# kowaalczyk/reformer-tts

Measured on AMD Instinct MI355X. Metric: mel-frames/sec training step, LJSpeech-shape batch, higher is better.
Workload: dtype bf16; 1 GPU; config/baseline.yml full Reformer-TTS training step (enc 3 / dec 3 layers, d=512, LSH 8 rounds, buckets 64/128), per-GPU batch 12, text 200->256, mel 1024x80; global_batch=12, parallelism=dp1, reversible_recompute=full

## Files before the change

### include/rtts.h

```cpp
#ifndef RTTS_H
#define RTTS_H

#include <stdint.h>

#ifdef __cplusplus
extern "C" {
#endif

#define RTTS_VERSION 1

int rtts_version(void);
const char* rtts_last_error(void);

int rtts_lsh_hash_sort(const void* qk, int64_t ld_qk, const float* rotations, int rot_rows,
                       int B, int H, int T, int dh, int n_hashes, int bucket_size,
                       int32_t* buckets, int32_t* st, int32_t* undo, void* stream);
int rtts_lsh_hash_sort_launches(int T);

int rtts_lsh_hash_sort_hf(const void* qk, int64_t ld_qk, const float* rotations, const uint8_t* mask,
                          int B, int H, int T, int dh, int n_hashes, int chunk, int n_buckets,
                          int32_t* buckets, int32_t* st, int32_t* undo, void* stream);

int rtts_lsh_attn_fwd(const void* qk, const void* v, int64_t ld, const int32_t* st, const uint8_t* mask,
                      int B, int H, int T, int dh, int n_hashes, int bucket_size, int causal,
// ... 109 lines not shown
int rtts_bn_act_bwd_sums(const float* y, const void* dz, int dz_halo, const float* mean, const float* rstd, const float* gamma,
                         const float* beta, int act, float drop_p, uint32_t seed, const uint32_t* seed_dev, int B, int L, int halo, int C,
                         float* sums, float* dgamma, float* dbeta, float* partial_ws, void* stream);
int rtts_bn_act_bwd_apply(const float* y, const void* dz, int dz_halo, const float* mean, const float* rstd, const float* gamma,
                          const float* beta, int act, float drop_p, uint32_t seed, const uint32_t* seed_dev, int B, int L, int halo, int C,
                          const float* sums, int64_t count, void* dy, int dy_lead, int64_t dy_rows, void* stream);
int rtts_tts_loss(const float* raw, const float* post, int64_t ld_mel, const float* tgt, const float* mask, const float* stop,
                  int64_t ld_stop, const float* tstop, int rows, int NM, int kind, float pos_weight, float w_raw, float w_post,
                  float w_stop, float* d_raw, float* d_post, int64_t ld_grad, float* d_stop, float* losses, float* partial_ws,
                  int padded_len, int valid_len, const float* res, int64_t ld_res, int halo, int dpost_lead, int64_t dpost_rows,
                  int64_t tgt_batch_stride, const int32_t* valid_len_dev, int64_t mask_batch_stride, int64_t tstop_batch_stride,
                  void* stream);
int rtts_heads_grad(const float* d_raw, const float* d_post, int dpost_lead, const float* dx0, int64_t ld_dx0, const float* d_stop,
                    int B, int L, int halo, int n_mels, int width, float* dheads, const float* scale_dev, void* stream);

#define RTTS_SEGMENTS_MAX 12
enum { RTTS_SEG_COPY_F32 = 0, RTTS_SEG_COPY_BF16 = 1, RTTS_SEG_ADD_F32 = 2, RTTS_SEG_CAST_F32_BF16 = 3 };
typedef struct {
    void* dst;
    const void* src;
    int64_t count;
    int32_t kind, reserved;
} rtts_segment;
int rtts_segments(const rtts_segment* jobs, int n, void* stream);

int rtts_pe_add(const void* y, const float* table, const float* alpha, float drop_p, uint32_t seed, const uint32_t* seed_dev,
                int T, int64_t M, int d, float* out, void* stream);
int rtts_pe_dalpha(const float* dy, const float* table, float drop_p, uint32_t seed, const uint32_t* seed_dev, int T, int64_t M,
                   int d, float* dalpha, float* partial_ws, void* stream);
int rtts_relu_drop(void* h, float drop_p, uint32_t seed, const uint32_t* seed_dev, int64_t n, void* stream);

int rtts_batch_masks(const int64_t* phonemes, int64_t ph_stride, int B, int Lp, int Lp_pad, const float* loss_mask, int64_t lm_bstride,
                     int64_t lm_rstride, int Lm, int Lm_pad, int n_mels, int64_t* pad_phonemes, uint8_t* phoneme_mask,
                     uint8_t* phoneme_pad_mask, uint8_t* frame_mask, void* stream);

int rtts_embedding_fwd(const int64_t* ids, const float* E, int rows, int C, int n_embeddings, float drop_p, uint32_t seed,
                       const uint32_t* seed_dev, float* out, void* stream);
int rtts_embedding_bwd(const int64_t* ids, const float* dx, int rows, int C, int n_embeddings, int padding_idx, float* dE,
                       float drop_p, uint32_t seed, const uint32_t* seed_dev, void* stream);
int rtts_embedding_bwd_strided(const int64_t* ids, const float* dx, int64_t batch_stride, int64_t row_stride, int L, int rows, int C,
                               int n_embeddings, int padding_idx, float* dE, float drop_p, uint32_t seed, const uint32_t* seed_dev, void* stream);

int rtts_gemm_tn(const void* a, int64_t lda, const void* b, int64_t ldb, int M, int N, int K, float* c, int64_t ldc,
                 int accumulate, float* slab_ws, int64_t slab_ws_floats, void* stream);

#define RTTS_GEMM_TN_MAX_GROUP 16
typedef struct {
    const void* a; int64_t lda;
    const void* b; int64_t ldb;
    float* c;      int64_t ldc;
    int32_t M, N, K, accumulate;
} rtts_gemm_tn_problem;
int rtts_gemm_tn_grouped(const rtts_gemm_tn_problem* problems, int n, float* slab_ws, int64_t slab_ws_floats, void* stream);

int rtts_gemm_nt(const void* a, int64_t lda, const void* w, int64_t ldw, int w_is_kn, int M, int N, int K, void* c,
                 int64_t ldc, const float* bias, int epilogue, const void* gate, int64_t ldg, float* colsum_partial,
                 void* stream);
int rtts_gemm_nt_partial_rows(int M, int N);
typedef struct {
    const void* a; int64_t lda;
    const void* w; int64_t ldw;
    void* c; int64_t ldc;
    const float* bias;
    const void* aux; int64_t ld_aux;
    float* aux_out;
    int32_t M, N, K, epilogue;
    int32_t T, H, accumulate, reserved;
} rtts_gemm_nt_problem;
#define RTTS_GEMM_NT_MAX_GROUP 4
int rtts_gemm_nt_grouped(const rtts_gemm_nt_problem* problems, int n, int w_is_kn, void* stream);
int rtts_debug_set_gemm_mode(int mode);
int64_t rtts_gemm_nt_gate_words(int M, int N);
int rtts_gemm_nt_gated(const void* a, int64_t lda, const void* w, int64_t ldw, int w_is_kn, int M, int N, int K, void* c,
                       int64_t ldc, const float* bias, int epilogue, uint64_t* gate_words, float* colsum_partial, void* stream);

int rtts_peak_copy(const void* src, void* dst, int64_t bytes, void* stream);
int rtts_comm_probe(const void* src, void* dst, int64_t bytes, int workgroups, int sleep, void* stream);
int rtts_debug_stamp(void* buf, int slot, void* stream);
int rtts_peak_mfma(float* sink, int workgroups, int iters, void* stream);

int rtts_sw_depthwise_k3(const float* x, const float* w, const float* bias, int B, int L, int C, void* y,
                         const float* edge_lo, const float* edge_hi, void* stream);
int rtts_sw_gate(const void* pw, const void* cond, int64_t ld_cond, int cond_offset, int upsample, int B, int L, int Lm, int C,
                 void* acts, void* stream);
int rtts_sw_coupling_inv(float* audio, int64_t ld_audio, const float* wn_out, int64_t rows, int half, void* stream);
int rtts_sw_depthwise_k3_seg(const float* x, const float* w, const float* bias, const int32_t* moff, int nseg, int upsample,
                             int64_t rows, int C, void* y, const float* edge_lo, const float* edge_hi, void* stream);
int rtts_sw_pack_mel(const float* mel, int64_t stride_b, int64_t stride_c, int64_t stride_t, int L, int n_mel, const int32_t* moff,
                     int nseg, int64_t rows, float* dst, int64_t ld_dst, void* stream);
int rtts_sw_coupling_inv1x1(const float* audio, int64_t ld_audio, const float* wn_out, int64_t ld_wn, const float* winv, int n,
                            int64_t rows, float* out, int64_t ld_out, void* stream);
int rtts_sw_coupling_fwd1x1(const float* x, int64_t ld_x, const float* wn_out, int64_t ld_wn, const float* w, int n_in, int n_early,
                            int64_t rows, float* out, int64_t ld_out, float* z, int64_t ld_z, int z_col, float* ls_row, void* stream);
int rtts_sw_nll_reduce(const float* z, int64_t ld_z, int C, const float* ls_row, const int32_t* moff, int nseg, int upsample, int64_t L,
                       int64_t rows, double* out, void* stream);
int rtts_sw_pack_audio(const float* src, int64_t n_src, const int64_t* start, const int32_t* moff, int nseg, int upsample, int C,
                       int64_t rows, float* dst, void* stream);
int rtts_sw_gate_bwd(const void* pw, const void* cond, int64_t ld_cond, int cond_offset, int upsample, int B, int L, int Lm, int C,
                     const void* dacts, void* dpw, void* dcond, int64_t ld_dcond, void* stream);
int rtts_sw_dwbn_bwd_partial_floats(int64_t rows, int C);
int rtts_sw_dwbn_bwd_sums(const float* h, const void* dy, const float* mean, const float* rstd, const float* gamma, const float* beta,
                          const float* w, int B, int L, int C, float* sums, float* partial_ws, void* stream);
int rtts_sw_dwbn_bwd_apply(const float* h, const void* dy, const float* mean, const float* rstd, const float* gamma, const float* beta,
                           const float* w, const float* sums, int B, int L, int C, float* dh, void* stream);
int rtts_sw_boundary_bwd_blocks(int64_t rows);
int rtts_sw_boundary_bwd(const float* x, int64_t ld_x, const float* wn_out, int64_t ld_wn, const float* w, int n_in, int n_early,
// ... 63 lines not shown
```

### reformer-tts_amd/_lib.py

```python
from __future__ import annotations

import ctypes as C
import os

_HERE = os.path.dirname(os.path.abspath(__file__))
LIB_PATH = os.environ.get("RTTS_LIB") or os.path.join(_HERE, "lib", "librtts_hip.so")

_i64, _i32, _vp, _f32, _u32 = C.c_int64, C.c_int, C.c_void_p, C.c_float, C.c_uint32

class GemmTnProblem(C.Structure):
    _fields_ = [("a", _vp), ("lda", _i64), ("b", _vp), ("ldb", _i64), ("c", _vp), ("ldc", _i64),
                ("M", C.c_int32), ("N", C.c_int32), ("K", C.c_int32), ("accumulate", C.c_int32)]


GEMM_TN_MAX_GROUP = 16


class GemmNtProblem(C.Structure):
    _fields_ = [("a", _vp), ("lda", _i64), ("w", _vp), ("ldw", _i64), ("c", _vp), ("ldc", _i64), ("bias", _vp), ("aux", _vp),
                ("ld_aux", _i64), ("aux_out", _vp), ("M", C.c_int32), ("N", C.c_int32), ("K", C.c_int32), ("epilogue", C.c_int32),
                ("T", C.c_int32), ("H", C.c_int32), ("accumulate", C.c_int32), ("reserved", C.c_int32)]


GEMM_NT_MAX_GROUP = 4


class ColsumJob(C.Structure):
    _fields_ = [("partial", _vp), ("out", _vp), ("nrows", C.c_int32), ("n", C.c_int32), ("ld", C.c_int32), ("reserved", C.c_int32)]


COLSUM_MAX_GROUP = 48


class Segment(C.Structure):
    _fields_ = [("dst", _vp), ("src", _vp), ("count", C.c_int64), ("kind", C.c_int32), ("reserved", C.c_int32)]


SEGMENTS_MAX = 12
SEG_COPY_F32, SEG_COPY_BF16, SEG_ADD_F32, SEG_CAST_F32_BF16 = 0, 1, 2, 3


class ConvPermJob(C.Structure):
    _fields_ = [("w", _vp), ("wp", _vp), ("Co", C.c_int32), ("Ci", C.c_int32), ("CP", C.c_int32), ("reserved", C.c_int32)]


CONV_PERM_MAX_GROUP = 8
SW_FACTOR_MAX_COUNT, SW_FACTOR_MAX_N = 16, 128

SIGNATURES = {
    "rtts_lsh_hash_sort": [_vp, _i64, _vp, _i32, _i32, _i32, _i32, _i32, _i32, _i32, _vp, _vp, _vp, _vp],
    "rtts_lsh_attn_fwd": [_vp, _vp, _i64, _vp, _vp, _i32, _i32, _i32, _i32, _i32, _i32, _i32, _vp, _vp, _f32, _u32, _vp, _vp],
    "rtts_lsh_hash_sort_launches": [_i32],
    "rtts_lsh_hash_sort_hf": [_vp, _i64, _vp, _vp, _i32, _i32, _i32, _i32, _i32, _i32, _i32, _vp, _vp, _vp, _vp],
    "rtts_lsh_attn_fwd_run_length": [_i32, _i32, _i32, _i32, _i32],
    "rtts_lsh_combine_fwd": [_vp, _vp, _i32, _i32, _i32, _i32, _i32, _vp, _i64, _vp, _vp],
    "rtts_lsh_bwd_delta": [_vp, _i64, _vp, _i64, _i32, _i32, _i32, _i32, _vp, _vp],
    "rtts_lsh_attn_bwd": [_vp, _vp, _i64, _vp, _vp, _vp, _i64, _vp, _vp, _i32, _i32, _i32, _i32, _i32, _i32, _i32, _vp, _vp, _vp, _f32, _u32, _vp,
                          _vp],
    "rtts_lsh_bwd_qk_slots": [],
    "rtts_lsh_attn_bwd_run_length": [_i32, _i32, _i32, _i32, _i32],
    "rtts_debug_set_walk": [_i32, _i32],
    "rtts_lsh_bwd_reduce": [_vp, _vp, _i32, _i32, _i32, _i32, _i32, _vp, _vp, _i64, _vp, _vp],
    "rtts_grad_clip_scale": [_vp, _i64, _f32, _f32, _vp, _vp, _vp],
    "rtts_ln_fwd": [_vp, _vp, _vp, _vp, _vp, _vp, _i32, _i32, _vp],
    "rtts_ln_bwd": [_vp, _vp, _vp, _vp, _vp, _vp, _vp, _vp, _vp, _i32, _i32, _vp, _vp, _f32, _u32, _vp, _vp],
    "rtts_ln_bwd_to": [_vp, _vp, _vp, _vp, _vp, _vp, _vp, _vp, _vp, _vp, _i32, _i32, _vp, _vp, _f32, _u32, _vp, _vp],
    "rtts_ln_bwd_join": [_vp, _vp, _vp, _vp, _vp, _vp, _vp, _vp, _vp, _vp, _vp, _i32, _i32, _vp, _vp, _f32, _u32, _vp, _vp],
    "rtts_cast_colsum": [_vp, _vp, _vp, _vp, _i32, _i32, _f32, _u32, _vp, _vp, _vp],
    "rtts_colsum_bf16": [_vp, _vp, _i64, _vp, _vp, _i32, _i32, _i32, _f32, _vp, _vp],
    "rtts_sum_streams": [_vp, _vp, _i64, _vp, _vp, _vp],
    "rtts_residual_epilogue": [_vp, _vp, _vp, _f32, _vp, _i64, _i32, _f32, _u32, _vp, _vp],
    "rtts_colsum_partial_rows": [_i32],
    "rtts_colsum_final_grouped": [C.POINTER(ColsumJob), _i32, _vp],
    "rtts_residual_ln": [_vp, _vp, _vp, _f32, _vp, _vp, _vp, _vp, _vp, _i32, _i32, _f32, _u32, _vp, _vp, _vp],
    "rtts_bias_act": [_vp, _vp, _i64, _i32, _i32, _vp],
    "rtts_cast_f32_bf16": [_vp, _vp, _i64, _vp],
    "rtts_xattn_fwd": [_vp, _i64, _vp, _i64, _vp, _i32, _i32, _i32, _i32, _i32, _vp, _i64, _vp, _f32, _u32, _vp, _vp],
    "rtts_xattn_bwd": [_vp, _i64, _vp, _i64, _vp, _vp, _i64, _vp, _vp, _i32, _i32, _i32, _i32, _i32, _vp, _i64, _vp, _f32, _u32, _vp, _vp, _vp],
    "rtts_xattn_key_chunks": [_i32],
    "rtts_xattn_bwd_key_chunks": [_i32, _i32],
    "rtts_xattn_probs_mean": [_vp, _i64, _vp, _i64, _vp, _vp, _i32, _i32, _i32, _i32, _i32, _vp, _i64, _vp],
    "rtts_sum_slabs": [_vp, _i32, _i64, _vp, _vp],
    "rtts_full_attn_max_t": [_i32],
    "rtts_full_attn_fwd": [_vp, _vp, _i64, _vp, _i32, _i32, _i32, _i32, _i32, _vp, _i64, _vp, _f32, _u32, _vp, _vp],
    "rtts_full_attn_bwd_workspace": [_i32, _i32, _i32, _i32],
    "rtts_full_attn_bwd": [_vp, _vp, _i64, _vp, _vp, _i64, _vp, _vp, _i32, _i32, _i32, _i32, _i32, _vp, _vp, _i64, _vp, _f32, _u32, _vp,
                           _vp],
    "rtts_conv1d_k5": [_vp, _i64, _vp, _i64, _i32, _i32, _i32, _i32, _vp, _i64, _vp, _i32, _vp],
    "rtts_to_halo": [_vp, _i64, _i64, _i32, _i32, _i32, _i32, _i32, _i32, _vp, _i32, _i64, _vp],
    "rtts_heads_grad": [_vp, _vp, _i32, _vp, _i64, _vp, _i32, _i32, _i32, _i32, _i32, _vp, _vp, _vp],
    "rtts_segments": [C.POINTER(Segment), _i32, _vp],
    "rtts_conv_w_perm": [_vp, _i32, _i32, _i32, _vp, _vp],
    "rtts_conv_dw_unperm": [_vp, _i32, _i32, _i32, _vp, _vp],
    "rtts_conv_w_perm_grouped": [C.POINTER(ConvPermJob), _i32, _vp],
    "rtts_conv_dw_unperm_grouped": [C.POINTER(ConvPermJob), _i32, _vp],
    "rtts_conv1d_k5_moments": [_vp, _i64, _vp, _i64, _i32, _i32, _i32, _vp, _i64, _i32, _i32, _i32, _vp, _vp],
    "rtts_bn_stats_from_partials": [_vp, _i32, _i32, _i32, _i32, _vp, _vp, _vp, _vp, _vp, _vp, _vp],
    "rtts_bn_stats": [_vp, _i32, _i32, _i32, _i32, _vp, _vp, _vp, _vp, _vp, _vp, _vp, _vp],
    "rtts_bn_act_fwd": [_vp, _vp, _vp, _vp, _vp, _i32, _f32, _u32, _vp, _i32, _i32, _i32, _i32, _vp, _i32, _i32, _i64, _vp],
    "rtts_bn_act_bwd": [_vp, _vp, _i32, _vp, _vp, _vp, _vp, _i32, _f32, _u32, _vp, _i32, _i32, _i32, _i32, _vp, _i32, _i64, _vp, _vp, _vp, _vp],
    "rtts_bn_moments": [_vp, _i32, _i32, _i32, _i32, _vp, _vp, _vp],
    "rtts_bn_from_moments": [_vp, _i64, _i32, _vp, _vp, _vp, _vp, _vp, _vp, _vp],
    "rtts_bn_act_bwd_sums": [_vp, _vp, _i32, _vp, _vp, _vp, _vp, _i32, _f32, _u32, _vp, _i32, _i32, _i32, _i32, _vp, _vp, _vp, _vp, _vp],
    "rtts_bn_act_bwd_apply": [_vp, _vp, _i32, _vp, _vp, _vp, _vp, _i32, _f32, _u32, _vp, _i32, _i32, _i32, _i32, _vp, _i64, _vp, _i32, _i64, _vp],
    "rtts_tts_loss": [_vp, _vp, _i64, _vp, _vp, _vp, _i64, _vp, _i32, _i32, _i32, _f32, _f32, _f32, _f32, _vp, _vp, _i64, _vp, _vp, _vp, _i32, _i32,
                      _vp, _i64, _i32, _i32, _i64, _i64, _vp, _i64, _i64, _vp],
    "rtts_pe_add": [_vp, _vp, _vp, _f32, _u32, _vp, _i32, _i64, _i32, _vp, _vp],
    "rtts_debug_stamp": [_vp, _i32, _vp],
    "rtts_batch_masks": [_vp, _i64, _i32, _i32, _i32, _vp, _i64, _i64, _i32, _i32, _i32, _vp, _vp, _vp, _vp, _vp],
    "rtts_pe_dalpha": [_vp, _vp, _f32, _u32, _vp, _i32, _i64, _i32, _vp, _vp, _vp],
    "rtts_relu_drop": [_vp, _f32, _u32, _vp, _i64, _vp],
    "rtts_embedding_bwd": [_vp, _vp, _i32, _i32, _i32, _i32, _vp, _f32, _u32, _vp, _vp],
    "rtts_embedding_bwd_strided": [_vp, _vp, _i64, _i64, _i32, _i32, _i32, _i32, _i32, _vp, _f32, _u32, _vp, _vp],
    "rtts_embedding_fwd": [_vp, _vp, _i32, _i32, _i32, _f32, _u32, _vp, _vp, _vp],
    "rtts_gemm_tn": [_vp, _i64, _vp, _i64, _i32, _i32, _i32, _vp, _i64, _i32, _vp, _i64, _vp],
    "rtts_gemm_tn_grouped": [C.POINTER(GemmTnProblem), _i32, _vp, _i64, _vp],
    "rtts_gemm_nt": [_vp, _i64, _vp, _i64, _i32, _i32, _i32, _i32, _vp, _i64, _vp, _i32, _vp, _i64, _vp, _vp],
    "rtts_gemm_nt_partial_rows": [_i32, _i32],
    "rtts_gemm_nt_grouped": [C.POINTER(GemmNtProblem), _i32, _i32, _vp],
    "rtts_debug_set_gemm_mode": [_i32],
    "rtts_gemm_nt_gate_words": [_i32, _i32],
    "rtts_gemm_nt_gated": [_vp, _i64, _vp, _i64, _i32, _i32, _i32, _i32, _vp, _i64, _vp, _i32, _vp, _vp, _vp],
    "rtts_peak_copy": [_vp, _vp, _i64, _vp],
    "rtts_comm_probe": [_vp, _vp, _i64, _i32, _i32, _vp],
    "rtts_peak_mfma": [_vp, _i32, _i32, _vp],
    "rtts_sw_depthwise_k3": [_vp, _vp, _vp, _i32, _i32, _i32, _vp, _vp, _vp, _vp],
    "rtts_sw_gate": [_vp, _vp, _i64, _i32, _i32, _i32, _i32, _i32, _i32, _vp, _vp],
    "rtts_sw_coupling_inv": [_vp, _i64, _vp, _i64, _i32, _vp],
    "rtts_sw_depthwise_k3_seg": [_vp, _vp, _vp, _vp, _i32, _i32, _i64, _i32, _vp, _vp, _vp, _vp],
    "rtts_sw_pack_mel": [_vp, _i64, _i64, _i64, _i32, _i32, _vp, _i32, _i64, _vp, _i64, _vp],
    "rtts_sw_coupling_inv1x1": [_vp, _i64, _vp, _i64, _vp, _i32, _i64, _vp, _i64, _vp],
    "rtts_sw_coupling_fwd1x1": [_vp, _i64, _vp, _i64, _vp, _i32, _i32, _i64, _vp, _i64, _vp, _i64, _i32, _vp, _vp],
    "rtts_sw_nll_reduce": [_vp, _i64, _i32, _vp, _vp, _i32, _i32, _i64, _i64, _vp, _vp],
    "rtts_sw_pack_audio": [_vp, _i64, _vp, _vp, _i32, _i32, _i32, _i64, _vp, _vp],
    "rtts_sw_gate_bwd": [_vp, _vp, _i64, _i32, _i32, _i32, _i32, _i32, _i32, _vp, _vp, _vp, _i64, _vp],
    "rtts_sw_dwbn_bwd_partial_floats": [_i64, _i32],
    "rtts_sw_dwbn_bwd_sums": [_vp, _vp, _vp, _vp, _vp, _vp, _vp, _i32, _i32, _i32, _vp, _vp, _vp],
    "rtts_sw_dwbn_bwd_apply": [_vp, _vp, _vp, _vp, _vp, _vp, _vp, _vp, _i32, _i32, _i32, _vp, _vp],
    "rtts_sw_boundary_bwd_blocks": [_i64],
    "rtts_sw_boundary_bwd": [_vp, _i64, _vp, _i64, _vp, _i32, _i32, _i64, _vp, _i64, _vp, _i64, _i32, _f32, _f32, _vp, _i64, _vp, _i64, _vp, _vp,
                             _vp],
    "rtts_sw_inv1x1_factor": [C.POINTER(_vp), C.POINTER(_i32), _i32, C.POINTER(_vp), _vp, _vp],
    "rtts_sw_draw_segments": [_vp, _i32, _i64, _vp, _vp, _i64, _vp, _i32, _vp, _i32, _vp, _u32, _vp, _i32, _i32, _i32, _i32, _i32, _vp, _vp, _i64,
                              _vp, _vp],
    "rtts_tts_collate": [_vp, _i64, _vp, _vp, _i64, _vp, _i32, _vp, _i32, _i32, _i32, _vp, _i32, _vp, _i32, _i32, _vp, _i32, _vp, _i32, _vp, _i32,
                         _vp, _f32, _u32, _vp],
    "rtts_infer_metrics_tiles": [_i32],
    "rtts_infer_metrics": [_vp, _i64, _i64, _i64, _i32, _vp, _vp, _i64, _i64, _i64, _vp, _i32, _vp, _vp, _vp, _i32, _i32, _i32, _i32, _vp, _vp, _vp,
                           _vp, _vp],
    "rtts_dtw_max_frames": [],
    "rtts_dtw_workspace_bytes": [_i32, _i32, _i32, _i32],
    "rtts_dtw_align": [_vp, _i64, _i64, _i64, _i32, _vp, _vp, _i64, _i64, _i64, _vp, _i32, _vp, _vp, _vp, _i32, _i32, _i32, _vp, _i32, _vp, _i64,
                       _i32, _vp, _vp, _vp, _vp],
    "rtts_adamw_step": [_vp, _vp, _vp, _vp, _vp, _i64, _vp, _vp, _f32, _f32, _f32, _f32, _vp, _vp],
    "rtts_mel_frames": [_i64, _i32],
    "rtts_mel_spectrogram": [_vp, C.POINTER(_i64), C.POINTER(_i64), _vp, _vp, _i32, _vp, _vp, _i32, _i32, _i32, _i32, _f32, _vp, _i64, _vp],
    "rtts_resample_len": [_i64, _i32, _i32],
    "rtts_resample": [_vp, _i32, _i32, C.POINTER(_i64), C.POINTER(_i64), _vp, _vp, _i32, _vp, _vp, _i32, _i32, _i32, _vp, _vp],
    "rtts_denoise": [_vp, C.POINTER(_i64), _vp, _i32, _vp, _vp, _vp, _f32, _i32, _i32, _vp, _vp],
    "rtts_gl_magnitudes": [_vp, _i64, _i64, _i64, _vp, C.POINTER(_i64), _vp, _i32, _vp, _i32, _i32, _i32, _vp, _i64, _vp],
    "rtts_gl_init": [_vp, _i64, C.POINTER(_i64), _vp, C.POINTER(_i64), _vp, _i32, _vp, _vp, _i32, _u32, _i32, _i32, _vp, _vp],
    "rtts_gl_step": [_vp, _vp, _f32, _vp, _i64, C.POINTER(_i64), _vp, C.POINTER(_i64), _vp, _i32, _vp, _vp, _i32, _i32, _vp, _vp],
}

_lib = None


class RttsError(RuntimeError):
    pass
# ... 82 lines not shown
```

### reformer-tts_amd/edges.py

```python
from __future__ import annotations

import threading
from typing import List

import torch

from . import _lib
from . import engine as _engine
from .engine import WEIGHT_EPOCH, _WS, _bf16, _grad, bf16_twin, cast_colsum, gemm, wgrad

from ._seeds import _seed_counter, seed_base


def _s() -> int:
    return torch.cuda.current_stream().cuda_stream


def _ws(device, c: int) -> torch.Tensor:
    key = ("edge", device, c, torch.cuda.current_stream(device).cuda_stream)
    if key not in _WS._cache:
        _WS._cache[key] = torch.empty((2 * 256 + 2) * c, dtype=torch.float32, device=device)
    return _WS._cache[key]


def _pad128(c: int) -> int:
    return -(-c // 128) * 128


class Halo:
    H, LEAD, TILE = 2, 8, 256

    def __init__(self, b: int, l: int):
        self.b, self.l = b, l
        self.p = l + 2 * self.H
        self.rows = b * self.p
        self.mp = -(-self.rows // self.TILE) * self.TILE
        self.alloc = self.mp + 2 * self.LEAD

    def new(self, c: int, device, dtype=torch.bfloat16) -> torch.Tensor:
        return torch.empty(self.alloc, c, dtype=dtype, device=device)

    def body(self, buf: torch.Tensor, shift: int = 0) -> torch.Tensor:
        return buf[self.LEAD + shift:self.LEAD + shift + self.mp]

    def valid(self, body: torch.Tensor) -> torch.Tensor:
        return body[:self.rows].view(self.b, self.p, -1)[:, self.H:self.H + self.l]


import os as _os
CONVS_PER_WGRAD_LAUNCH = int(_os.environ.get("RTTS_CONVS_PER_WGRAD", "4"))


def flush_conv_wgrad(queue=None) -> None:
    queue = _engine._queue() if queue is None else queue
    q = queue.conv_gemms
    wide = [p for p in q if p[0][7] % 256 == 0 and p[0][8] % 256 == 0]
    rest = [p for p in q if not (p[0][7] % 256 == 0 and p[0][8] % 256 == 0)]
    del q[:]
    for part in (wide, rest):
        while part:
            chunk = part[:_lib.GEMM_TN_MAX_GROUP]
            del part[:len(chunk)]
            arr = (_lib.GemmTnProblem * len(chunk))()
            for dst, (fields, _keep) in zip(arr, chunk):
                dst.a, dst.lda, dst.b, dst.ldb, dst.c, dst.ldc, dst.M, dst.N, dst.K, dst.accumulate = fields
            ws = _engine._slab_ws(chunk[0][1][0].device, queue.stream)
            _lib.call("rtts_gemm_tn_grouped", arr, len(chunk), ws.data_ptr(), ws.numel(), queue.stream)


def flush_conv_dw(queue=None) -> None:
    queue = _engine._queue() if queue is None else queue
    flush_conv_wgrad(queue)
    pending = list(queue.conv_items)
    del queue.conv_items[:]
    for chunk in _engine.launch_groups(pending, _lib.CONV_PERM_MAX_GROUP,
                                       lambda a, b: _engine.spans_overlap(a[4].data_ptr(), 20 * a[1] * a[2], b[4].data_ptr(), 20 * b[1] * b[2])):
        jobs = (_lib.ConvPermJob * len(chunk))()
        for j, (dwp, co, ci, cp, gw) in zip(jobs, chunk):
            j.w, j.wp, j.Co, j.Ci, j.CP = dwp.data_ptr(), gw.data_ptr(), co, ci, cp
        _lib.call("rtts_conv_dw_unperm_grouped", jobs, len(chunk), queue.stream)


class ConvK5:

    instances = None

    def __init__(self, conv: torch.nn.Conv1d):
        self.conv = conv
        self.co, self.ci = conv.out_channels, conv.in_channels
        self.cp = _pad128(self.ci)
        self.cop = _pad128(self.co)
        self._wp = None
        self._wp_version = None
        if ConvK5.instances is None:
            import weakref
            ConvK5.instances = weakref.WeakSet()
        ConvK5.instances.add(self)

    def _version(self):
        w = self.conv.weight
        return (w._version, WEIGHT_EPOCH[0], w.data_ptr())

    @staticmethod
    def refresh_all(device) -> None:
        stale = [c for c in (ConvK5.instances or ()) if c.conv.weight.device == device and c._wp_version != c._version()]
        for i in range(0, len(stale), _lib.CONV_PERM_MAX_GROUP):
            chunk = stale[i:i + _lib.CONV_PERM_MAX_GROUP]
            jobs = (_lib.ConvPermJob * len(chunk))()
            for j, c in zip(jobs, chunk):
                if c._wp is None or c._wp.device != device:
                    c._wp = torch.zeros(c.cop, 5 * c.cp, dtype=torch.bfloat16, device=device)
                j.w, j.wp, j.Co, j.Ci, j.CP = c.conv.weight.data_ptr(), c._wp.data_ptr(), c.co, c.ci, c.cp
            _lib.call("rtts_conv_w_perm_grouped", jobs, len(chunk), _s())
            for c in chunk:
                c._wp_version = c._version()

    def weight_perm(self) -> torch.Tensor:
        w = self.conv.weight
        ver = (w._version, WEIGHT_EPOCH[0], w.data_ptr())
        if self._wp is None or self._wp_version != ver or self._wp.device != w.device:
            if self._wp is None or self._wp.device != w.device:
                self._wp = torch.zeros(self.cop, 5 * self.cp, dtype=torch.bfloat16, device=w.device)
            _lib.call("rtts_conv_w_perm", w.data_ptr(), self.co, self.ci, self.cp, self._wp.data_ptr(), _s())
            self._wp_version = ver
        return self._wp

    def forward(self, xh: torch.Tensor, g: Halo, bias=None) -> torch.Tensor:
        y = torch.empty(g.mp, self.cop, dtype=torch.float32, device=xh.device)
        wp = self.weight_perm()
        _lib.call("rtts_conv1d_k5", g.body(xh).data_ptr(), self.cp, wp.data_ptr(), 5 * self.cp, 0, g.mp, self.cop, self.cp, y.data_ptr(),
                  self.cop, None if bias is None else bias.data_ptr(), 1, _s())
        return y

    def forward_moments(self, xh: torch.Tensor, g: Halo):
        y = torch.empty(g.mp, self.cop, dtype=torch.float32, device=xh.device)
        nrows = _lib.load().rtts_gemm_nt_partial_rows(g.mp, self.cop)
        if nrows <= 0:
            raise _lib.RttsError(f"rtts_conv1d_k5_moments: no tile shape for {g.mp} x {self.cop}")
        partial = torch.empty(nrows, 2 * self.cop, dtype=torch.float32, device=xh.device)
        _lib.call("rtts_conv1d_k5_moments", g.body(xh).data_ptr(), self.cp, self.weight_perm().data_ptr(), 5 * self.cp, g.mp, self.cop, self.cp,
                  y.data_ptr(), self.cop, g.b, g.l, g.H, partial.data_ptr(), _s())
        return y, partial, nrows

    def backward(self, dyh: torch.Tensor, xh: torch.Tensor, g: Halo, need_dx: bool = True, dx_f32: bool = False):
        dev = dyh.device
        dwp = torch.empty(self.cop, 5 * self.cp, dtype=torch.float32, device=dev)
        dyb = g.body(dyh)
        dwq = _engine._queue()
        for k in range(5):
            xs, ck = g.body(xh, k - 2), dwp[:, k * self.cp:(k + 1) * self.cp]
            dwq.conv_gemms.append(((dyb.data_ptr(), self.cop, xs.data_ptr(), self.cp, ck.data_ptr(), 5 * self.cp, g.mp, self.cop, self.cp, 0),
                              (dyh, xh, dwp)))
        if len(dwq.conv_gemms) >= 5 * CONVS_PER_WGRAD_LAUNCH:
            flush_conv_wgrad(dwq)
        dwq.conv_items.append((dwp, self.co, self.ci, self.cp, _grad(self.conv.weight)))
        if len(dwq.conv_items) >= _lib.CONV_PERM_MAX_GROUP:
            flush_conv_dw(dwq)
        else:
            from .engine import _queue_final_flush
            _queue_final_flush()
        if not need_dx:
            return None
        dx = torch.empty(g.mp, self.cp, dtype=torch.float32 if dx_f32 else torch.bfloat16, device=dev)
        _lib.call("rtts_conv1d_k5", dyb.data_ptr(), self.cop, self.weight_perm().data_ptr(), 5 * self.cp, 1, g.mp, self.cp, self.cop,
                  dx.data_ptr(), self.cp, None, int(dx_f32), _s())
        return dx


SYNC_BN = None
CONV_MOMENTS = _os.environ.get("RTTS_CONV_MOMENTS", "1") != "0"


class ConvBNAct:

    def __init__(self, conv, bn, act: int, p: float):
        self.c = ConvK5(conv)
        self.bn, self.act, self.p = bn, act, float(p)

    def forward(self, xh, g: Halo, plain_out: bool = False):
        fused = SYNC_BN is None and CONV_MOMENTS
        y, partial, nrows = self.c.forward_moments(xh, g) if fused else (self.c.forward(xh, g), None, 0)
        c = y.shape[1]
        dev = y.device
        mean = torch.empty(c, dtype=torch.float32, device=dev)
        rstd = torch.empty(c, dtype=torch.float32, device=dev)
        bn = self.bn
        if fused:
            _lib.call("rtts_bn_stats_from_partials", partial.data_ptr(), nrows, g.b, g.l, c, mean.data_ptr(), rstd.data_ptr(),
                      bn.running_mean.data_ptr(), bn.running_var.data_ptr(), self.c.conv.bias.data_ptr(), bn.num_batches_tracked.data_ptr(), _s())
        elif SYNC_BN is None:
            _lib.call("rtts_bn_stats", y.data_ptr(), g.b, g.l, g.H, c, mean.data_ptr(), rstd.data_ptr(), bn.running_mean.data_ptr(),
                      bn.running_var.data_ptr(), self.c.conv.bias.data_ptr(), bn.num_batches_tracked.data_ptr(), _ws(dev, c).data_ptr(), _s())
        else:
            import torch.distributed as dist
            mom = torch.empty(2 * c + 1, dtype=torch.float32, device=dev)
            _lib.call("rtts_bn_moments", y.data_ptr(), g.b, g.l, g.H, c, mom.data_ptr(), _ws(dev, c).data_ptr(), _s())
            mom[2 * c:].fill_(float(g.b * g.l))
            dist.all_reduce(mom, group=SYNC_BN)
            _lib.call("rtts_bn_from_moments", mom.data_ptr(), 0, c, mean.data_ptr(), rstd.data_ptr(), bn.running_mean.data_ptr(),
                      bn.running_var.data_ptr(), self.c.conv.bias.data_ptr(), bn.num_batches_tracked.data_ptr(), _s())
        seed = next(_seed_counter) * 2654435761 % (1 << 32)
        if plain_out:
            z = torch.empty(g.b * g.l, c, dtype=torch.bfloat16, device=dev)
            zargs = (0, 0, g.b * g.l)
        else:
            z = g.new(c, dev)
            zargs = (1, g.LEAD, g.alloc)
        _lib.call("rtts_bn_act_fwd", y.data_ptr(), mean.data_ptr(), rstd.data_ptr(), bn.weight.data_ptr(), bn.bias.data_ptr(), self.act,
                  self.p, seed, seed_base(dev).data_ptr(), g.b, g.l, g.H, c, z.data_ptr(), *zargs, _s())
        return z, (xh, y, mean, rstd, seed)

    def backward(self, dz, dz_halo: bool, saved, g: Halo, need_dx=True, dx_f32=False):
        xh, y, mean, rstd, seed = saved
        c = y.shape[1]
        bn = self.bn
        dy = g.new(c, y.device)
# ... 394 lines not shown
```

### reformer-tts_amd/engine.py

```python
from __future__ import annotations

from typing import List, Optional

import os

import torch

from . import _lib, ops
from ._seeds import next_seed, seed_base
from .model.lsh_attention import LSHSelfAttention


STASH_ATTENTION = True
STASH_BLOCK_OUTPUT = True
STASH_PROJECTIONS = True
STASH_STREAMS = True
_NO_G = object()


def _streams_kept() -> bool:
    return STASH_STREAMS and STASH_ATTENTION and STASH_BLOCK_OUTPUT and STASH_PROJECTIONS


RECOMPUTE_MODES = ("full", "attention-stash", "output-stash", "projection-stash", "stash")
# ... 56 lines not shown
    return m if m is not None else p.detach().to(torch.bfloat16)


def bf16_twin(x: torch.Tensor) -> Optional[torch.Tensor]:
    tw = getattr(x, "_rtts_bf16", None)
    if tw is None or tw[1] != x._version or tw[0].device != x.device:
        return None
    return tw[0]


def _adjacent(a: torch.Tensor, b: torch.Tensor) -> bool:
    return (a.untyped_storage().data_ptr() == b.untyped_storage().data_ptr() and a.is_contiguous() and b.is_contiguous()
            and a.data_ptr() + a.numel() * a.element_size() == b.data_ptr())


def _grad(p: torch.Tensor) -> torch.Tensor:
    if p.grad is None:
        p.grad = torch.zeros_like(p)
    return p.grad


class _WS:
    _cache = {}

    @classmethod
    def partial(cls, device, d: int) -> torch.Tensor:
        key = (device, d, torch.cuda.current_stream(device).cuda_stream)
        if key not in cls._cache:
            cls._cache[key] = torch.empty(2 * 256 * d, dtype=torch.float32, device=device)
        return cls._cache[key]


def ln_fwd(x, norm):
    m, d = x.shape
    xn = torch.empty(m, d, dtype=torch.bfloat16, device=x.device)
    mean = torch.empty(m, dtype=torch.float32, device=x.device)
    rstd = torch.empty(m, dtype=torch.float32, device=x.device)
    _lib.call("rtts_ln_fwd", x.data_ptr(), norm.weight.data_ptr(), norm.bias.data_ptr(), xn.data_ptr(), mean.data_ptr(),
              rstd.data_ptr(), m, d, _s())
    return xn, mean, rstd


DEFER_COLSUM = True


class _Queue:

    def __init__(self, device: int, stream: int):
        self.device, self.stream = device, stream
        self.colsums = []
        self.wgrads = []
        self.conv_gemms = []
        self.conv_items = []
        self.flush_queued = False

    def __len__(self):
        return len(self.colsums) + len(self.wgrads) + len(self.conv_gemms) + len(self.conv_items)

    def clear(self):
        del self.colsums[:], self.wgrads[:], self.conv_gemms[:], self.conv_items[:]
        self.flush_queued = False


_QUEUES = {}
_QLOCK = __import__("threading").RLock()


def _queue() -> _Queue:
    key = (torch.cuda.current_device(), _s())
    q = _QUEUES.get(key)
    if q is None:
        with _QLOCK:
            q = _QUEUES.setdefault(key, _Queue(*key))
    return q


def _all_queues(keys=None):
    with _QLOCK:
        if keys is None:
            return list(_QUEUES.values())
        return [_QUEUES[k] for k in keys if k in _QUEUES]


def drop_stream_state(device_index: int, stream: int) -> None:
    with _QLOCK:
        q = _QUEUES.get((device_index, stream))
        if q is not None and not len(q):
            del _QUEUES[(device_index, stream)]
    for key in [k for k in _WS._cache if isinstance(k, tuple) and k[-1] == stream and
                (getattr(k[0], "index", None) == device_index or getattr(k[1], "index", None) == device_index)]:
        del _WS._cache[key]


def _partial_rows(m: int) -> int:
    return min((m + 3) // 4, 256)


def _queue_colsum(partial: torch.Tensor, offset_floats: int, rows: int, d: int, out: torch.Tensor, ld: int = 0):
    _queue().colsums.append((partial, offset_floats, rows, d, out, ld))
    _queue_final_flush()


def launch_groups(items, cap: int, overlap):
    groups, cur = [], []
    for it in items:
        if len(cur) == cap or any(overlap(it, c) for c in cur):
            groups.append(cur)
            cur = []
        cur.append(it)
    if cur:
        groups.append(cur)
    return groups

# ... 936 lines not shown
```

Measured before the change: 1.936 million mel-frames/s.

## Add fused five-tap conv1d weight-gradient kernel with split-K and grouped launches

Adds a dedicated HIP kernel for the conv1d k=5 weight gradient. It computes all five taps from a single staged dY/X tile pipeline, using async global-to-LDS loads, a ring buffer for X with halo rows, and MFMA accumulation. It replaces five separate TN GEMMs per conv plus the permute/accumulate pass. Split-K partial results go to a slab and a reduce kernel adds them into dw; when the slab is too small the kernel adds directly into dw. This adds a large hand-scheduled kernel with hard-coded waitcnt encodings, and it now becomes the default path.

```diff
diff --git a/include/rtts.h b/include/rtts.h
--- a/include/rtts.h
+++ b/include/rtts.h
@@ -185,6 +185,16 @@
     int32_t M, N, K, accumulate;
 } rtts_gemm_tn_problem;
 int rtts_gemm_tn_grouped(const rtts_gemm_tn_problem* problems, int n, float* slab_ws, int64_t slab_ws_floats, void* stream);
+
+#define RTTS_CONV_WGRAD_MAX_GROUP 8
+typedef struct {
+    const void* dy; int64_t lddy;
+    const void* x;  int64_t ldx;
+    float* dw;
+    int M, Co, Ci, CoP, CiP;
+} rtts_conv_wgrad_job;
+int rtts_conv1d_k5_wgrad_grouped(const rtts_conv_wgrad_job* jobs, int n, float* slab_ws, int64_t slab_ws_floats, void* stream);
+int rtts_debug_set_conv_wgrad_split(int split);
 
 int rtts_gemm_nt(const void* a, int64_t lda, const void* w, int64_t ldw, int w_is_kn, int M, int N, int K, void* c,
                  int64_t ldc, const float* bias, int epilogue, const void* gate, int64_t ldg, float* colsum_partial,
diff --git a/reformer-tts_amd/_lib.py b/reformer-tts_amd/_lib.py
--- a/reformer-tts_amd/_lib.py
+++ b/reformer-tts_amd/_lib.py
@@ -45,6 +45,14 @@
 
 
 CONV_PERM_MAX_GROUP = 8
+
+
+class ConvWgradJob(C.Structure):
+    _fields_ = [("dy", _vp), ("lddy", _i64), ("x", _vp), ("ldx", _i64), ("dw", _vp),
+                ("M", C.c_int32), ("Co", C.c_int32), ("Ci", C.c_int32), ("CoP", C.c_int32), ("CiP", C.c_int32)]
+
+
+CONV_WGRAD_MAX_GROUP = 8
 SW_FACTOR_MAX_COUNT, SW_FACTOR_MAX_N = 16, 128
 
 SIGNATURES = {
@@ -115,6 +123,8 @@
     "rtts_embedding_fwd": [_vp, _vp, _i32, _i32, _i32, _f32, _u32, _vp, _vp, _vp],
     "rtts_gemm_tn": [_vp, _i64, _vp, _i64, _i32, _i32, _i32, _vp, _i64, _i32, _vp, _i64, _vp],
     "rtts_gemm_tn_grouped": [C.POINTER(GemmTnProblem), _i32, _vp, _i64, _vp],
+    "rtts_conv1d_k5_wgrad_grouped": [C.POINTER(ConvWgradJob), _i32, _vp, _i64, _vp],
+    "rtts_debug_set_conv_wgrad_split": [_i32],
     "rtts_gemm_nt": [_vp, _i64, _vp, _i64, _i32, _i32, _i32, _i32, _vp, _i64, _vp, _i32, _vp, _i64, _vp, _vp],
     "rtts_gemm_nt_partial_rows": [_i32, _i32],
     "rtts_gemm_nt_grouped": [C.POINTER(GemmNtProblem), _i32, _i32, _vp],
diff --git a/reformer-tts_amd/csrc/conv_wgrad.h b/reformer-tts_amd/csrc/conv_wgrad.h
--- /dev/null
+++ b/reformer-tts_amd/csrc/conv_wgrad.h
@@ -0,0 +1,81 @@
+#pragma once
+
+#if defined(__HIPCC__) || defined(__CUDACC__)
+#define CW_HD __host__ __device__
+#else
+#define CW_HD
+#endif
+
+#define CW_TAPS 5
+#define CW_RS 32
+#define CW_NST 4
+#define CW_NXS 5
+#define CW_AHEAD 3
+#define CW_BCO 128
+#define CW_BCI 64
+#define CW_NW 4
+#define CW_ROWA (CW_BCO * 2)
+#define CW_ROWX (CW_BCI * 2)
+#define CW_STAGE_A (CW_RS * CW_ROWA)
+#define CW_STAGE_X (CW_RS * CW_ROWX)
+#define CW_RING_X (CW_NXS * CW_STAGE_X)
+#define CW_DMA_PER_GROUP 3
+
+CW_HD constexpr int cw_run_stages(int st_all, int split, int sp) { return st_all / split + (sp < st_all % split ? 1 : 0); }
+CW_HD constexpr int cw_run_first(int st_all, int split, int sp) {
+    return sp * (st_all / split) + (sp < st_all % split ? sp : st_all % split);
+}
+
+CW_HD constexpr int cw_a_slot(int s) { return s % CW_NST; }
+CW_HD constexpr int cw_x_slot(int t) { return t % CW_NXS; }
+
+CW_HD constexpr int cw_a_key(int row) { return row & 3; }
+CW_HD constexpr int cw_x_key(int row) { return (row >> 1) & 1; }
+
+CW_HD constexpr int cw_a_dma_row(int w, int i, int lane) { return 8 * w + 4 * i + (lane >> 4); }
+CW_HD constexpr int cw_a_dma_col(int w, int i, int lane) {
+    return ((((lane & 15) >> 2) ^ cw_a_key(cw_a_dma_row(w, i, lane))) << 6) + ((lane & 3) << 4);
+}
+CW_HD constexpr int cw_x_dma_row(int w, int lane) { return 8 * w + (lane >> 3); }
+CW_HD constexpr int cw_x_dma_col(int w, int lane) {
+    return ((((lane & 7) >> 2) ^ cw_x_key(cw_x_dma_row(w, lane))) << 6) + ((lane & 3) << 4);
+}
+CW_HD constexpr int cw_x_src_row(int m_begin, int t, int row, int M) {
+    return (m_begin + CW_RS * t + row - 2) < (M + 1) ? (m_begin + CW_RS * t + row - 2) : (M + 1);
+}
+
+CW_HD constexpr int cw_lane_hh(int lane) { return lane >> 5; }
+CW_HD constexpr int cw_lane_trq(int lane) { return (lane & 15) >> 2; }
+CW_HD constexpr int cw_lane_trp(int lane) { return lane & 3; }
+CW_HD constexpr int cw_lane_trc(int lane) { return (lane >> 4) & 1; }
+CW_HD constexpr int cw_a_frag_off(int wn, int t, int lane) {
+    const int row = 8 * cw_lane_hh(lane) + cw_lane_trq(lane);
+    const int cb = (wn * 64 + t * 32 + 16 * cw_lane_trc(lane) + 4 * cw_lane_trp(lane)) * 2;
+    return row * CW_ROWA + ((((cb >> 6) ^ cw_a_key(row)) << 6) | (cb & 63));
+}
+CW_HD constexpr int cw_x_frag_off(int wk, int k, int lane) {
+    const int row = 8 * cw_lane_hh(lane) + cw_lane_trq(lane) + k;
+    const int cb = (wk * 32 + 16 * cw_lane_trc(lane) + 4 * cw_lane_trp(lane)) * 2;
+    return row * CW_ROWX + ((((cb >> 6) ^ cw_x_key(row)) << 6) | (cb & 63));
+}
+CW_HD constexpr int cw_x_wrap(int ring_off) { return ring_off >= CW_RING_X ? ring_off - CW_RING_X : ring_off; }
+CW_HD constexpr int cw_x_read_off(int s, int wk, int k, int ks, int second, int lane) {
+    return cw_x_wrap(cw_x_slot(s) * CW_STAGE_X + cw_x_frag_off(wk, k, lane) + (16 * ks + 4 * second) * CW_ROWX);
+}
+CW_HD constexpr int cw_a_read_off(int s, int wn, int t, int ks, int second, int lane) {
+    return cw_a_slot(s) * CW_STAGE_A + cw_a_frag_off(wn, t, lane) + (16 * ks + 4 * second) * CW_ROWA;
+}
+
+CW_HD constexpr int cw_group_of_a(int s) { return s; }
+CW_HD constexpr int cw_group_of_x(int t) { return t - 1; }
+CW_HD constexpr int cw_issue_stage(int g) { return g < CW_AHEAD ? -1 : g - CW_AHEAD; }
+CW_HD constexpr int cw_ready_stage(int g) { return g < 0 ? 0 : g; }
+CW_HD constexpr int cw_wait_count(int s, int nstage) {
+    return CW_DMA_PER_GROUP * ((nstage - 1 - s) < (CW_AHEAD - 1) ? (nstage - 1 - s) : (CW_AHEAD - 1));
+}
+CW_HD constexpr int cw_first_read_of_x(int t) { return t > 0 ? t - 1 : 0; }
+CW_HD constexpr int cw_last_read_of_x(int t, int nstage) { return t < nstage ? t : nstage - 1; }
+
+static_assert(CW_NST == CW_AHEAD + 1, "dY slot of group s + AHEAD is the one stage s - 1 left");
+static_assert(CW_NXS == CW_AHEAD + 2, "X slot of group s + AHEAD (X stage s + AHEAD + 1) is the one X stage s - 1 left");
+static_assert(CW_RING_X % (4 * CW_ROWX) == 0 && CW_STAGE_A % (4 * CW_ROWA) == 0, "the keys' period divides stage and ring");
diff --git a/reformer-tts_amd/csrc/conv_wgrad.hip b/reformer-tts_amd/csrc/conv_wgrad.hip
--- /dev/null
+++ b/reformer-tts_amd/csrc/conv_wgrad.hip
@@ -0,0 +1,275 @@
+#include "rtts_common.h"
+#include "conv_wgrad.h"
+
+struct CwJob {
+    const bf16_t* dy;
+    const bf16_t* x;
+    float* slab;
+    float* dw;
+    int64_t lddy, ldx;
+    int M, Co, Ci, CoP, CiP, split;
+    int wg_start;
+    int rb_start;
+    int direct;
+};
+struct CwGroup {
+    CwJob j[RTTS_CONV_WGRAD_MAX_GROUP];
+    int n;
+};
+
+__global__ __launch_bounds__(64 * CW_NW, 2) void conv_wgrad_kernel(const CwGroup grp) {
+    __shared__ __attribute__((aligned(1024))) unsigned char As[CW_NST * CW_STAGE_A];
+    __shared__ __attribute__((aligned(1024))) unsigned char Xs[CW_RING_X];
+
+    int pi = 0;
+#pragma unroll
+    for (int i = 1; i < RTTS_CONV_WGRAD_MAX_GROUP; ++i)
+        if (i < grp.n && (int)blockIdx.x >= grp.j[i].wg_start) pi = i;
+    const CwJob& P = grp.j[pi];
+    const bf16_t* __restrict__ dy = P.dy;
+    const bf16_t* __restrict__ x = P.x;
+    const int64_t lddy = P.lddy, ldx = P.ldx;
+    const int M = P.M, CoP = P.CoP, CiP = P.CiP, split = P.split;
+    const int tiles_ci = CiP / CW_BCI, tiles = (CoP / CW_BCO) * tiles_ci;
+    const int blk = (int)xcd_remap((uint32_t)((int)blockIdx.x - P.wg_start), (uint32_t)(tiles * split));
+    const int sp = blk / tiles, tile = blk % tiles;
+    const int co0 = (tile / tiles_ci) * CW_BCO, ci0 = (tile % tiles_ci) * CW_BCI;
+    const int st_all = M / CW_RS;
+    const int nstage = cw_run_stages(st_all, split, sp);
+    const int m_begin = cw_run_first(st_all, split, sp) * CW_RS;
+
+    const int tid = threadIdx.x, lane = tid & 63, wave = __builtin_amdgcn_readfirstlane(tid >> 6);
+    const int wn = wave >> 1, wk = wave & 1;
+    const int hh = lane >> 5;
+
+    const bf16_t* srcA[2];
+#pragma unroll
+    for (int i = 0; i < 2; ++i)
+        srcA[i] = dy + ((size_t)m_begin + cw_a_dma_row(wave, i, lane)) * lddy + co0 + (cw_a_dma_col(wave, i, lane) >> 1);
+    const int xrow = cw_x_dma_row(wave, lane);
+    const bf16_t* srcX = x + ci0 + (cw_x_dma_col(wave, lane) >> 1);
+#define CW_ISSUE_X(t_)                                                                                                   \
+    __builtin_amdgcn_global_load_lds(                                                                                    \
+        (const __attribute__((address_space(1))) void*)(srcX + (int64_t)cw_x_src_row(m_begin, (t_), xrow, M) * ldx),     \
+        (RTTS_LDS void*)(Xs + cw_x_slot(t_) * CW_STAGE_X + 8 * wave * CW_ROWX), 16, 0, 0)
+#define CW_ISSUE(g_)                                                                                                     \
+    do {                                                                                                                 \
+        const int grp_ = (g_);                    \
+        _Pragma("unroll") for (int ii_ = 0; ii_ < 2; ++ii_)                                                              \
+            __builtin_amdgcn_global_load_lds(                                                                            \
+                (const __attribute__((address_space(1))) void*)(srcA[ii_] + (size_t)grp_ * CW_RS * lddy),                \
+                (RTTS_LDS void*)(As + cw_a_slot(grp_) * CW_STAGE_A + (8 * wave + 4 * ii_) * CW_ROWA), 16, 0, 0);         \
+        CW_ISSUE_X(grp_ + 1);                                                                                            \
+    } while (0)
+
+    f32x16 acc[2][CW_TAPS];
+#pragma unroll
+    for (int t = 0; t < 2; ++t)
+#pragma unroll
+        for (int k = 0; k < CW_TAPS; ++k) acc[t][k] = (f32x16){0};
+
+    uint32_t offA[2], offX[CW_TAPS];
+#pragma unroll
+    for (int t = 0; t < 2; ++t) offA[t] = (uint32_t)cw_a_frag_off(wn, t, lane);
+#pragma unroll
+    for (int k = 0; k < CW_TAPS; ++k) offX[k] = (uint32_t)cw_x_frag_off(wk, k, lane);
+    const uint32_t as0 = (uint32_t)(uintptr_t)(RTTS_LDS unsigned char*)As;
+    const uint32_t xs0 = (uint32_t)(uintptr_t)(RTTS_LDS unsigned char*)Xs;
+
+    static_assert(CW_AHEAD == 3 && CW_DMA_PER_GROUP == 3, "the counted waits below");
+    CW_ISSUE_X(0);
+#pragma unroll
+    for (int i = 0; i < CW_AHEAD; ++i)
+        if (i < nstage) CW_ISSUE(i);
+    for (int s = 0; s < nstage; ++s) {
+        const int left = cw_wait_count(s, nstage);
+        if (left >= 6) __builtin_amdgcn_s_waitcnt(0x0F76);
+        else if (left == 3) __builtin_amdgcn_s_waitcnt(0x0F73);
+        else __builtin_amdgcn_s_waitcnt(0x0F70);
+        asm volatile("s_barrier" ::: "memory");
+        if (s + CW_AHEAD < nstage) CW_ISSUE(s + CW_AHEAD);
+        const uint32_t abase = as0 + cw_a_slot(s) * CW_STAGE_A;
+        const uint32_t xbase = xs0 + cw_x_slot(s) * CW_STAGE_X;
+        short4v al[2][2], ah[2][2], xl[2][CW_TAPS], xh[2][CW_TAPS];
+#define CW_TR(dst, addr, off) asm volatile("ds_read_b64_tr_b16 %0, %1 offset:%2" : "=v"(dst) : "v"(addr), "n"(off))
+#pragma unroll
+        for (int ks = 0; ks < 2; ++ks) {
+#pragma unroll
+            for (int t = 0; t < 2; ++t) {
+                const uint32_t ad = abase + offA[t];
+                if (ks == 0) { CW_TR(al[0][t], ad, 0); CW_TR(ah[0][t], ad, 4 * CW_ROWA); }
+                else { CW_TR(al[1][t], ad, 16 * CW_ROWA); CW_TR(ah[1][t], ad, 20 * CW_ROWA); }
+            }
+#pragma unroll
+            for (int k = 0; k < CW_TAPS; ++k) {
+                const uint32_t ad = xbase + offX[k];
+                if (ks == 0) { CW_TR(xl[0][k], ad, 0); CW_TR(xh[0][k], ad, 4 * CW_ROWX); }
+                else {
+                    CW_TR(xl[1][k], ad, 16 * CW_ROWX);
+                    uint32_t aw = ad + 20 * CW_ROWX;
+                    aw = aw >= xs0 + CW_RING_X ? aw - CW_RING_X : aw;
+                    CW_TR(xh[1][k], aw, 0);
+                }
+            }
+        }
+#undef CW_TR
+        static_assert(CW_TAPS == 5, "operand lists of the waits below");
+#define CW_OPS(ks)                                                                                                        \
+    "+v"(al[ks][0]), "+v"(ah[ks][0]), "+v"(al[ks][1]), "+v"(ah[ks][1]), "+v"(xl[ks][0]), "+v"(xh[ks][0]), "+v"(xl[ks][1]), \
+        "+v"(xh[ks][1]), "+v"(xl[ks][2]), "+v"(xh[ks][2]), "+v"(xl[ks][3]), "+v"(xh[ks][3]), "+v"(xl[ks][4]), "+v"(xh[ks][4])
+        asm volatile("s_waitcnt lgkmcnt(0)" : CW_OPS(0));
+        asm volatile("" : CW_OPS(1));
+#undef CW_OPS
+#pragma unroll
+        for (int ks = 0; ks < 2; ++ks) {
+            bf16x8 af[2], xf[CW_TAPS];
+#pragma unroll
+            for (int t = 0; t < 2; ++t) {
+                const short4v lo = al[ks][t], hi = ah[ks][t];
+                const __attribute__((ext_vector_type(8))) short f = {lo[0], lo[1], lo[2], lo[3], hi[0], hi[1], hi[2], hi[3]};
+                af[t] = __builtin_bit_cast(bf16x8, f);
+            }
+#pragma unroll
+            for (int k = 0; k < CW_TAPS; ++k) {
+                const short4v lo = xl[ks][k], hi = xh[ks][k];
+                const __attribute__((ext_vector_type(8))) short f = {lo[0], lo[1], lo[2], lo[3], hi[0], hi[1], hi[2], hi[3]};
+                xf[k] = __builtin_bit_cast(bf16x8, f);
+            }
+#pragma unroll
+            for (int k = 0; k < CW_TAPS; ++k)
+#pragma unroll
+                for (int t = 0; t < 2; ++t) acc[t][k] = __builtin_amdgcn_mfma_f32_32x32x16_bf16(af[t], xf[k], acc[t][k], 0, 0, 0);
+        }
+    }
+#undef CW_ISSUE
+#undef CW_ISSUE_X
+
+    const int ci = ci0 + wk * 32 + (lane & 31);
+    if (P.direct) {
+        float* __restrict__ dw = P.dw;
+        const int Co = P.Co, Ci = P.Ci;
+#pragma unroll
+        for (int t = 0; t < 2; ++t)
+#pragma unroll
+            for (int k = 0; k < CW_TAPS; ++k)
+#pragma unroll
+                for (int e = 0; e < 16; ++e) {
+                    const int co = co0 + wn * 64 + t * 32 + 4 * hh + (e & 3) + 8 * (e >> 2);
+                    if (co < Co && ci < Ci) dw[((size_t)co * Ci + ci) * CW_TAPS + k] += acc[t][k][e];
+                }
+        return;
+    }
+    const size_t plane = (size_t)CoP * CiP;
+    float* __restrict__ dst = P.slab + (size_t)sp * CW_TAPS * plane;
+#pragma unroll
+    for (int t = 0; t < 2; ++t)
+#pragma unroll
+        for (int k = 0; k < CW_TAPS; ++k)
+#pragma unroll
+            for (int e = 0; e < 16; ++e) {
+                const int co = co0 + wn * 64 + t * 32 + 4 * hh + (e & 3) + 8 * (e >> 2);
+                dst[k * plane + (size_t)co * CiP + ci] = acc[t][k][e];
+            }
+}
+
+__global__ __launch_bounds__(256) void conv_wgrad_reduce_kernel(const CwGroup grp) {
+    int pi = 0;
+#pragma unroll
+    for (int i = 1; i < RTTS_CONV_WGRAD_MAX_GROUP; ++i)
+        if (i < grp.n && (int)blockIdx.x >= grp.j[i].rb_start) pi = i;
+    const CwJob& P = grp.j[pi];
+    if (P.direct) return;
+    const size_t plane = (size_t)P.CoP * P.CiP;
+    const size_t e = (size_t)((int)blockIdx.x - P.rb_start) * blockDim.x + threadIdx.x;
+    if (e >= plane) return;
+    const int co = (int)(e / P.CiP), ci = (int)(e % P.CiP);
+    if (co >= P.Co || ci >= P.Ci) return;
+    const float* __restrict__ slab = P.slab + e;
+    float s[CW_TAPS];
+#pragma unroll
+    for (int k = 0; k < CW_TAPS; ++k) s[k] = slab[k * plane];
+    for (int t = 1; t < P.split; ++t) {
+        const float* __restrict__ sl = slab + (size_t)t * CW_TAPS * plane;
+#pragma unroll
+        for (int k = 0; k < CW_TAPS; ++k) s[k] += sl[k * plane];
+    }
+    float* __restrict__ d = P.dw + ((size_t)co * P.Ci + ci) * CW_TAPS;
+#pragma unroll
+    for (int k = 0; k < CW_TAPS; ++k) d[k] += s[k];
+}
+
+static std::atomic<int> cw_forced_split{0};
+
+extern "C" int rtts_debug_set_conv_wgrad_split(int split) {
+    RTTS_REQUIRE(split >= 0, "rtts_debug_set_conv_wgrad_split: split must be >= 0 (0 = the library's choice)");
+    cw_forced_split.store(split, std::memory_order_relaxed);
+    return 0;
+}
+
+extern "C" int rtts_conv1d_k5_wgrad_grouped(const rtts_conv_wgrad_job* jobs, int n, float* slab_ws, int64_t slab_ws_floats, void* stream) {
+    RTTS_ENTER(stream);
+    RTTS_REQUIRE(jobs && n > 0 && n <= RTTS_CONV_WGRAD_MAX_GROUP, "rtts_conv1d_k5_wgrad_grouped: 1..%d jobs", RTTS_CONV_WGRAD_MAX_GROUP);
+    RTTS_REQUIRE(slab_ws_floats >= 0 && (((uintptr_t)slab_ws) & 15) == 0, "rtts_conv1d_k5_wgrad_grouped: bad slab workspace");
+    long long total_tiles = 0;
+    for (int i = 0; i < n; ++i) {
+        const rtts_conv_wgrad_job& q = jobs[i];
+        RTTS_REQUIRE(q.dy && q.x && q.dw, "rtts_conv1d_k5_wgrad: null pointer");
+        RTTS_REQUIRE(q.M > 0 && q.M % 64 == 0 && q.CoP > 0 && q.CiP > 0 && q.CoP % 128 == 0 && q.CiP % 128 == 0,
+                     "rtts_conv1d_k5_wgrad: need M %% 64 == 0, CoP %% 128 == 0, CiP %% 128 == 0 (got M=%d CoP=%d CiP=%d)", q.M, q.CoP, q.CiP);
+        RTTS_REQUIRE(q.Co > 0 && q.Ci > 0 && q.Co <= q.CoP && q.Ci <= q.CiP, "rtts_conv1d_k5_wgrad: need 0 < Co <= CoP, 0 < Ci <= CiP");
+        RTTS_REQUIRE(q.lddy >= q.CoP && q.ldx >= q.CiP && q.lddy % 8 == 0 && q.ldx % 8 == 0, "rtts_conv1d_k5_wgrad: bad leading dimensions");
+        RTTS_REQUIRE((((uintptr_t)q.dy | (uintptr_t)q.x) & 15) == 0 && (((uintptr_t)q.dw) & 3) == 0,
+                     "rtts_conv1d_k5_wgrad: dy and x must be 16-byte aligned, dw 4-byte aligned");
+        total_tiles += (long long)(q.CoP / CW_BCO) * (q.CiP / CW_BCI);
+    }
+    for (int i = 1; i < n; ++i)
+        for (int j = 0; j < i; ++j) {
+            const uintptr_t bi = (uintptr_t)jobs[i].dw, ei = bi + (uintptr_t)jobs[i].Co * jobs[i].Ci * CW_TAPS * sizeof(float);
+            const uintptr_t bj = (uintptr_t)jobs[j].dw, ej = bj + (uintptr_t)jobs[j].Co * jobs[j].Ci * CW_TAPS * sizeof(float);
+            RTTS_REQUIRE(bi >= ej || bj >= ei,
+                         "rtts_conv1d_k5_wgrad_grouped: jobs %d and %d write overlapping dw (launch them one after the other)", j, i);
+        }
+    RTTS_REQUIRE(total_tiles < (1 << 20), "rtts_conv1d_k5_wgrad_grouped: too many tiles");
+    const int forced = cw_forced_split.load(std::memory_order_relaxed);
+    int want = forced > 0 ? forced : (int)(512 / total_tiles);
+    if (want < 1) want = 1;
+    auto split_of = [&](const rtts_conv_wgrad_job& q, int w) {
+        const int stages = q.M / CW_RS;
+        const int cap = forced > 0 ? stages : (stages / 4 > 0 ? stages / 4 : 1);
+        return w < cap ? w : cap;
+    };
+    auto slab_need = [&](int w) {
+        size_t need = 0;
+        for (int i = 0; i < n; ++i) need += (size_t)split_of(jobs[i], w) * CW_TAPS * jobs[i].CoP * jobs[i].CiP;
+        return need;
+    };
+    const size_t have = slab_ws ? (size_t)slab_ws_floats : 0;
+    while (want > 1 && slab_need(want) > have) --want;
+    CwGroup grp;
+    grp.n = n;
+    int wg = 0, rb = 0;
+    size_t used = 0;
+    for (int i = 0; i < n; ++i) {
+        const rtts_conv_wgrad_job& q = jobs[i];
+        CwJob& P = grp.j[i];
+        const int split = split_of(q, want);
+        const size_t slab = (size_t)split * CW_TAPS * q.CoP * q.CiP;
+        P.dy = (const bf16_t*)q.dy; P.x = (const bf16_t*)q.x; P.dw = q.dw;
+        P.lddy = q.lddy; P.ldx = q.ldx;
+        P.M = q.M; P.Co = q.Co; P.Ci = q.Ci; P.CoP = q.CoP; P.CiP = q.CiP; P.split = split;
+        P.wg_start = wg;
+        P.rb_start = rb;
+        P.direct = used + slab > have;
+        P.slab = P.direct ? nullptr : slab_ws + used;
+        wg += (q.CoP / CW_BCO) * (q.CiP / CW_BCI) * split;
+        if (!P.direct) {
+            used += slab;
+            rb += (q.CoP * q.CiP + 255) / 256;
+        }
+    }
+    hipStream_t s = (hipStream_t)stream;
+    hipLaunchKernelGGL(conv_wgrad_kernel, dim3(wg), dim3(64 * CW_NW), 0, s, grp);
+    if (rb > 0) hipLaunchKernelGGL(conv_wgrad_reduce_kernel, dim3(rb), dim3(256), 0, s, grp);
+    RTTS_LAUNCH_CHECK("rtts_conv1d_k5_wgrad_grouped");
+    return 0;
+}
diff --git a/reformer-tts_amd/edges.py b/reformer-tts_amd/edges.py
--- a/reformer-tts_amd/edges.py
+++ b/reformer-tts_amd/edges.py
@@ -49,10 +49,22 @@
 
 import os as _os
 CONVS_PER_WGRAD_LAUNCH = int(_os.environ.get("RTTS_CONVS_PER_WGRAD", "4"))
+CONV_WGRAD = _os.environ.get("RTTS_CONV_WGRAD", "taps")
+if CONV_WGRAD not in ("taps", "gemm_tn"):
+    raise ValueError(f"RTTS_CONV_WGRAD must be 'taps' or 'gemm_tn', not {CONV_WGRAD!r}")
 
 
 def flush_conv_wgrad(queue=None) -> None:
     queue = _engine._queue() if queue is None else queue
+    pending = list(queue.conv_wgrads)
+    del queue.conv_wgrads[:]
+    for chunk in _engine.launch_groups(pending, _lib.CONV_WGRAD_MAX_GROUP,
+                                       lambda a, b: _engine.spans_overlap(a[0][4], 20 * a[0][6] * a[0][7], b[0][4], 20 * b[0][6] * b[0][7])):
+        jobs = (_lib.ConvWgradJob * len(chunk))()
+        for j, (fields, _keep) in zip(jobs, chunk):
+            j.dy, j.lddy, j.x, j.ldx, j.dw, j.M, j.Co, j.Ci, j.CoP, j.CiP = fields
+        ws = _engine._slab_ws(chunk[0][1][0].device, queue.stream)
+        _lib.call("rtts_conv1d_k5_wgrad_grouped", jobs, len(chunk), ws.data_ptr(), ws.numel(), queue.stream)
     q = queue.conv_gemms
     wide = [p for p in q if p[0][7] % 256 == 0 and p[0][8] % 256 == 0]
     rest = [p for p in q if not (p[0][7] % 256 == 0 and p[0][8] % 256 == 0)]
@@ -144,6 +156,17 @@
 
     def backward(self, dyh: torch.Tensor, xh: torch.Tensor, g: Halo, need_dx: bool = True, dx_f32: bool = False):
         dev = dyh.device
+        if CONV_WGRAD == "taps":
+            dwq = _engine._queue()
+            gw = _grad(self.conv.weight)
+            dwq.conv_wgrads.append(((g.body(dyh).data_ptr(), self.cop, g.body(xh).data_ptr(), self.cp, gw.data_ptr(), g.mp, self.co, self.ci,
+                                     self.cop, self.cp), (dyh, xh, gw)))
+            if len(dwq.conv_wgrads) >= CONVS_PER_WGRAD_LAUNCH:
+                flush_conv_wgrad(dwq)
+            else:
+                from .engine import _queue_final_flush
+                _queue_final_flush()
+            return self._input_grad(dyh, g, dx_f32) if need_dx else None
         dwp = torch.empty(self.cop, 5 * self.cp, dtype=torch.float32, device=dev)
         dyb = g.body(dyh)
         dwq = _engine._queue()
@@ -159,9 +182,11 @@
         else:
             from .engine import _queue_final_flush
             _queue_final_flush()
-        if not need_dx:
-            return None
-        dx = torch.empty(g.mp, self.cp, dtype=torch.float32 if dx_f32 else torch.bfloat16, device=dev)
+        return self._input_grad(dyh, g, dx_f32) if need_dx else None
+
+    def _input_grad(self, dyh: torch.Tensor, g: Halo, dx_f32: bool):
+        dyb = g.body(dyh)
+        dx = torch.empty(g.mp, self.cp, dtype=torch.float32 if dx_f32 else torch.bfloat16, device=dyh.device)
         _lib.call("rtts_conv1d_k5", dyb.data_ptr(), self.cop, self.weight_perm().data_ptr(), 5 * self.cp, 1, g.mp, self.cp, self.cop,
                   dx.data_ptr(), self.cp, None, int(dx_f32), _s())
         return dx
diff --git a/reformer-tts_amd/engine.py b/reformer-tts_amd/engine.py
--- a/reformer-tts_amd/engine.py
+++ b/reformer-tts_amd/engine.py
@@ -132,13 +132,14 @@
         self.wgrads = []
         self.conv_gemms = []
         self.conv_items = []
+        self.conv_wgrads = []
         self.flush_queued = False
 
     def __len__(self):
-        return len(self.colsums) + len(self.wgrads) + len(self.conv_gemms) + len(self.conv_items)
+        return len(self.colsums) + len(self.wgrads) + len(self.conv_gemms) + len(self.conv_items) + len(self.conv_wgrads)
 
     def clear(self):
-        del self.colsums[:], self.wgrads[:], self.conv_gemms[:], self.conv_items[:]
+        del self.colsums[:], self.wgrads[:], self.conv_gemms[:], self.conv_items[:], self.conv_wgrads[:]
         self.flush_queued = False
 
 
```

New measurement: 1.955 million mel-frames/s (median of 6 runs). No clear change (+1.0%).
